# cadia-lvl/ss_asr

Measured on AMD Instinct MI355X. Metric: train-step utterances/sec on 80-dim mel, higher is better.
Workload: dtype f32; 1 GPU; BASELINE.json configs[1]: one ASRTrainer.exec iteration (GPU batch assembly from the HBM-resident corpus + engine.ASRTrainStep), ~10h synthetic Malromur-shape fbanks (8000 utts, <=800 frames, 80-dim), batch 32 per GPU, bucketed by length, LAS 256/256/128, tf_rate 0.9, Adadelta; global_batch=32, max_frames=800, parallelism=dp1, matrix_products=fp32 as 6 bf16 MFMAs on exact 3-way operand split, fp32 accumulate

## Files before the change

### ss_asr_amd/csrc/common.h

```cpp
#pragma once
#include <hip/hip_runtime.h>
#include <stdint.h>

typedef float f32x4 __attribute__((ext_vector_type(4)));

#define SSASR_OK 0
#define SSASR_EARG (-1)

#define SSASR_LAUNCH_CHECK()                         \
  do {                                               \
    hipError_t e__ = hipGetLastError();              \
    if (e__ != hipSuccess) return (int)e__;          \
  } while (0)

#define SSASR_HIP(call)                              \
  do {                                               \
    hipError_t e__ = (call);                         \
    if (e__ != hipSuccess) return (int)e__;          \
  } while (0)

struct RowMap {
  int64_t ld;
  int64_t inner;
  int64_t so;
// ... 130 lines not shown
  int no_fused_input;
  int bptt_halves_off;
  int bptt_reserve_kb;
  int no_persistent_decoder;
  int no_persistent_decoder_bwd;
  int delay_fwd, delay_bwd, delay_bwd_ksplit;
  int gemm_tile;
  int gemm_trace_lo, gemm_trace_hi;
  int gemm_wide;
  int gemm_bf16;
  int gemm_x6;
  int gemm_kcat;
  int no_windows;
  int bptt_one_launch;
  int wgrad_fused;
  int last_seg_pct;
  int tail_inline;
  int no_residency_check;
  int test_drop_tile;
  int test_drop_attn_slice;
  int test_drop_dec_slice;
  int attn_rph;
  int no_tsave;
};
const SsasrOptions& ssasr_options();
int64_t ssasr_resident_capacity(const void* kernel, int threads, size_t dyn_lds);
size_t ssasr_gemm_min_lds_bytes();
size_t ssasr_lds_reservation_against_gemm(const void* kernel);
bool ssasr_bptt_ksplit_ok(int64_t S, int64_t N, int64_t H, int dirs);
extern "C" int64_t ssasr_bilstm_bwd_gx_floats(int64_t S, int64_t N, int64_t H);
int ssasr_launch_colsum(const float* m, int64_t rows, int cols, int64_t ld, float* out, hipStream_t st,
                        float* out2 = nullptr);
```

### ss_asr_amd/csrc/decoder.hip

```cpp
#include "../../include/ssasr.h"
#include "attn_kernels.h"
#include "rnn_kernels.h"
#ifdef SSASR_TRACE_BUILD
constexpr int DTR_STEPS = 64, DTR_SLOTS = 8, DTR_WG = 256;
__device__ unsigned long long g_dtrace[DTR_WG * DTR_STEPS * DTR_SLOTS];
#define SSASR_DTRACE(step, slot) do { if (threadIdx.x == 0 && (step) < DTR_STEPS) { \
  unsigned long long t_; asm volatile("s_memrealtime %0\n\ts_waitcnt lgkmcnt(0)" : "=s"(t_) :: "memory"); \
  g_dtrace[(blockIdx.x * DTR_STEPS + (step)) * DTR_SLOTS + (slot)] = t_; } } while (0)
#endif
#include "decoder_persistent.h"
#include "decoder_long.h"
#include "decoder_bwd_persistent.h"
#include <cstdlib>

extern "C" int ssasr_abi_version(void) { return 16; }
#ifdef SSASR_TRACE_BUILD
extern "C" int ssasr_debug_dtrace(void* dst, size_t bytes) {
  SSASR_HIP(hipMemcpyFromSymbol(dst, HIP_SYMBOL(g_dtrace), bytes));
  return SSASR_OK;
}
#endif

extern "C" int64_t ssasr_decoder_bwd_chain_floats(int64_t U, int64_t B, int64_t T, int64_t A, int64_t E, int64_t D) {
  if (A != PD_A || E != PD_E || D != PD_D || B <= 0 || B > 32 || T <= 0 || U <= 0) return 0;
  if (chain_slices(T) == 0 || chain_slices(T) * B > CB_MAXATT) return 0;
  if (chain_xc_floats(U) * sizeof(float) >= (1ull << 31)) return 0;
  return (int64_t)(U * B * A + ((U * B + 63) & ~(int64_t)63) + chain_xa_floats(U) + chain_xc_floats(U) +
                   chain_xu_floats(U, T) + U * B * 4 * D);
}

namespace {
bool dec_grid_fits(const void* kernel, int threads, size_t dyn_lds, int64_t workgroups);
bool dec_long_taken(int64_t B, int64_t T, int64_t A, int64_t E, int64_t D, int64_t V) {
  const SsasrOptions& opt = ssasr_options();
  if (A != PD_A || E != PD_E || D != PD_D || V <= 0 || V > 64 || !pl_shape_ok(B, T)) return false;
  if (opt.no_persistent || opt.no_persistent_decoder) return false;
  const void* fn = reinterpret_cast<const void*>(decoder_fwd_long_kernel);
  if (hipFuncSetAttribute(fn, hipFuncAttributeMaxDynamicSharedMemorySize, (int)decoder_long_lds()) != hipSuccess) return false;
  return dec_grid_fits(fn, 512, decoder_long_lds(), (int64_t)pl_ns(T) * B + PL_NCMP);
}
}

extern "C" int64_t ssasr_decoder_fwd_part_floats(int64_t B, int64_t T, int64_t A, int64_t E, int64_t D, int64_t V) {
  return dec_long_taken(B, T, A, E, D, V) ? pl_part_floats(B, T) : 0;
}

extern "C" int ssasr_attn_precompute_fwd(const float* feat, const float* w_psi, const float* b_psi,
                                         int64_t rows, int64_t E, int64_t A, float* comp,
                                         void* stream) {
  if (!feat || !w_psi || !comp || rows <= 0 || E <= 0 || A <= 0) return SSASR_EARG;
  GemmDesc g{};
// ... 371 lines not shown
  int rc;
  const int64_t rows = U * B;
  const RowMap logit_rows{0, B, V, U * V};

  {
    GemmDesc m{};
    m.A = g.dlogits; m.ma = logit_rows;
    m.B = d.w_ct; m.mb = rm_dense(D);
    m.C = g.ws_dh2; m.mc = rm_dense(D);
    m.M = (int)rows; m.N = (int)D; m.K = (int)V; m.ta = 0; m.tb = 1;
    m.alpha = 1.f; m.beta = 0.f; m.splitk = 1; m.batch = 1;
    if ((rc = ssasr_launch_gemm(m, st))) return rc;
  }

  const bool cell2_first = g.ws_gx && g.ws_sync && ssasr_bilstm_bwd_gx_floats(U, B, D) > 0 &&
                           !opt.no_persistent && !opt.no_persistent_decoder;
  const bool cell2_direct = cell2_first && ssasr_bptt_ksplit_ok(U, B, D, 1);
  bool chain = cell2_first && g.ws_chain && ssasr_decoder_bwd_chain_floats(U, B, T, A, E, D) > 0 &&
               !opt.no_persistent_decoder_bwd;
  const int nsl = chain_slices(T);
  const void* chain_fn = nsl == 6 ? reinterpret_cast<const void*>(decoder_bwd_chain_kernel<6>)
                       : nsl == 4 ? reinterpret_cast<const void*>(decoder_bwd_chain_kernel<4>)
                                  : reinterpret_cast<const void*>(decoder_bwd_chain_kernel<2>);
  if (chain) {
    const size_t lds = chain_lds_bytes((int)T);
    SSASR_HIP(hipFuncSetAttribute(chain_fn, hipFuncAttributeMaxDynamicSharedMemorySize, (int)lds));
    chain = dec_grid_fits(chain_fn, 320, lds, nsl * B + 64);
  }
  if (!chain) {
    if ((rc = ssasr_launch_transpose(d.w_phi, d.w_phi_t, (int)A, (int)D, st))) return rc;
    if ((rc = ssasr_launch_transpose(d.w_ih1, g.ws_t_ih1, (int)(4 * D), (int)(D + E), st))) return rc;
    if ((rc = ssasr_launch_transpose(d.w_hh1, g.ws_t_hh1, (int)(4 * D), (int)D, st))) return rc;
  }
  if (!cell2_first && (rc = ssasr_launch_transpose(d.w_ih2, g.ws_t_ih2, (int)(4 * D), (int)D, st))) return rc;
  if (!cell2_direct && (rc = ssasr_launch_transpose(d.w_hh2, g.ws_t_hh2, (int)(4 * D), (int)D, st))) return rc;

  dim3 cgrid = cell_bwd_grid(D, 1, B), cblock(256);
  float* dc1 = g.ws_dc;
  float* dc2 = g.ws_dc + 2 * B * D;
  if (cell2_first) {
    if ((rc = ssasr_launch_bptt_persistent(cell2_direct ? nullptr : g.ws_t_hh2, d.gates2, d.c2, g.ws_dh2, B * D, D,
                                           nullptr, g.ws_gx, g.ws_sync, U, B, D, 1, st, 0, 0, nullptr,
                                           cell2_direct ? d.w_hh2 : nullptr, nullptr, armed && cell2_direct)))
      return rc;
    GemmDesc m{};
    m.A = d.gates2; m.ma = rm_dense(4 * D);
    m.B = d.w_ih2; m.mb = rm_dense(D);
    m.C = g.ws_dh2; m.mc = rm_dense(D);
    m.M = (int)rows; m.N = (int)D; m.K = (int)(4 * D); m.ta = 0; m.tb = 1;
    m.alpha = 1.f; m.beta = 0.f; m.splitk = 1; m.batch = 1;
    if (((rows + 63) / 64) * ((D + 63) / 64) < 192) {
      SSASR_HIP(hipMemsetAsync(g.ws_dh2, 0, sizeof(float) * rows * D, st));
      m.splitk = 4;
    }
    if ((rc = ssasr_launch_gemm(m, st))) return rc;
  }
  if (chain) {
    float* wsV = g.ws_chain;
    float* wsS = wsV + U * B * A;
    float* xa = wsS + ((U * B + 63) & ~(int64_t)63);
    float* xc = xa + chain_xa_floats(U);
    float* xu = xc + chain_xc_floats(U);
    float* dg1 = xu + chain_xu_floats(U, T);
    {
      GemmDesc m{};
      m.A = d.att; m.ma = rm_dense(T); m.sa = U * T;
      m.B = d.comp; m.mb = rm_dense(A); m.sb = T * A;
      m.C = wsV; m.mc = rm_dense(B * A); m.sc = A;
      m.M = (int)U; m.N = (int)A; m.K = (int)T; m.ta = 0; m.tb = 1;
      m.alpha = 1.f; m.beta = 0.f; m.splitk = 1; m.batch = (int)B;
      if ((rc = ssasr_launch_gemm(m, st))) return rc;
    }
    if (!armed)
      SSASR_HIP(hipMemsetD32Async((hipDeviceptr_t)xa, (int)PERSIST_SENTINEL,
                                  chain_xa_floats(U) + chain_xc_floats(U) + chain_xu_floats(U, T), st));
    DecBwdChain c{};
    c.gates1 = d.gates1; c.dg1 = dg1; c.c1 = d.c1; c.add1 = g.ws_dh2; c.att = d.att; c.q = d.q; c.feat = d.feat;
    c.comp = d.comp; c.enc_len = d.enc_len; c.V = wsV; c.w_hh1 = d.w_hh1; c.w_ih1 = d.w_ih1;
    c.w_phi = d.w_phi; c.dctx = g.ws_dctx; c.de = g.ws_de; c.dqpre = g.ws_dqpre; c.ssum = wsS;
    c.xa = xa; c.xc = xc; c.xu = xu; c.status = g.ws_sync + 5;
    c.B = (int)B; c.T = (int)T; c.U = (int)U;
    const size_t lds = chain_lds_bytes((int)T);
    const dim3 cgrid_chain((unsigned)(nsl * B + 64));
    if (nsl == 6) hipLaunchKernelGGL(decoder_bwd_chain_kernel<6>, cgrid_chain, dim3(320), lds, st, c);
    else if (nsl == 4) hipLaunchKernelGGL(decoder_bwd_chain_kernel<4>, cgrid_chain, dim3(320), lds, st, c);
    else hipLaunchKernelGGL(decoder_bwd_chain_kernel<2>, cgrid_chain, dim3(320), lds, st, c);
    hipLaunchKernelGGL(chain_de_fixup_kernel, dim3(256), dim3(256), 0, st, g.ws_de, d.att, wsS, (int)B, (int)U, (int)T,
                       reinterpret_cast<float4*>(d.gates1), reinterpret_cast<const float4*>(dg1), U * B * D,
                       g.ws_dqpre, (int)(B * A));
    SSASR_LAUNCH_CHECK();
  }
  for (int64_t t = U - 1; t >= 0 && !chain; --t) {
    const int64_t i = U - 1 - t;
    const bool last = (t == U - 1);
    CellBwdPair p2{};
    if (!cell2_first) {
      CellBwd& c = p2.d[0];
      int ns = 0;
      if (!last) {
        seg_set(c.sl, ns++, d.gates2 + (t + 1) * B * 4 * D, 4 * D, g.ws_t_hh2, 4 * D, (int)(4 * D));
        c.dc_in = dc2 + (i & 1) * B * D;
      }
      c.sl.nseg = ns;
      c.add1 = g.ws_dh2 + t * B * D; c.ld1 = D;
      c.gates = d.gates2 + t * B * 4 * D; c.dgates = d.gates2 + t * B * 4 * D;
      c.c_prev = t ? d.c2 + (t - 1) * B * D : nullptr;
// ... 124 lines not shown
```

### ss_asr_amd/csrc/decoder_bwd_persistent.h

```cpp
#pragma once
#include "decoder_persistent.h"

namespace {

constexpr int CB_XU_SLOTS = 34;
constexpr int CB_MAXATT = 192;
__host__ __device__ inline int cb_xu_step(int nsl) { return 2 * nsl * CB_XU_SLOTS * 16 * 4; }
__host__ __device__ inline int chain_slices(int64_t T) { return T <= 128 ? 2 : T <= 256 ? 4 : T <= 384 ? 6 : 0; }

struct DecBwdChain {
  const float* gates1;
  float* dg1;
  const float* c1;
  const float* add1;
  const float* att;
  const float* q;
  const float* feat;
  const float* comp;
  const int32_t* enc_len;
  const float* V;
  const float* w_hh1;
  const float* w_ih1;
  const float* w_phi;
  float* dctx;
  float* de;
  float* dqpre;
  float* ssum;
  float* xa;
  float* xc;
  float* xu;
  int* status;
  int B, T, U;
};

__host__ __device__ inline size_t chain_xa_floats(int64_t U) { return (size_t)U * 2 * 16 * 16 * 256; }
__host__ __device__ inline size_t chain_xc_floats(int64_t U) { return (size_t)U * 2 * 16 * 32 * 256; }
__host__ __device__ inline size_t chain_xu_floats(int64_t U, int64_t T) { return (size_t)U * cb_xu_step(chain_slices(T)); }
inline size_t chain_lds_bytes(int T) {
  const int nsl = chain_slices(T);
  const size_t att = ((size_t)((T + nsl - 1) / nsl) * PD_E + PD_E + 8 * PD_A + 16) * sizeof(float);
  const size_t cell = (4 * 64 * 4 + 2 * 7 * 64 * 4 + 4 * 64 * 4 + 8 * 4 * 16 * 4) * sizeof(float);
  return att > cell ? att : cell;
}

__global__ void chain_de_fixup_kernel(float* de, const float* att, const float* ssum, int B, int U, int T,
                                      float4* gates1, const float4* dg1, int64_t ng4, float* dqpre0, int nq) {
  const int64_t tid = blockIdx.x * (int64_t)blockDim.x + threadIdx.x, nth = (int64_t)gridDim.x * blockDim.x;
  for (int64_t i = tid; i < ng4; i += nth) gates1[i] = dg1[i];
  for (int64_t i = tid; i < nq; i += nth) dqpre0[i] = 0.f;
  const int64_t n = (int64_t)B * U * T;
  for (int64_t i = tid; i < n; i += nth) {
    const int64_t b = i / ((int64_t)U * T);
    const int64_t t = (i / T) % U;
    de[i] = t > 0 ? de[i] - att[i] * ssum[t * B + b] : 0.f;
  }
}

#ifndef SSASR_WPACE_UP
#define SSASR_WPACE_UP 12
#endif
#ifndef SSASR_WPACE_CLEAN
#define SSASR_WPACE_CLEAN 2
#endif
#ifndef SSASR_WPACE_DOWN
#define SSASR_WPACE_DOWN 2
#endif
#ifndef SSASR_WPACE_INIT
#define SSASR_WPACE_INIT 100
#endif
#ifndef SSASR_WPACE_INIT_ATT
#define SSASR_WPACE_INIT_ATT 120
#endif
struct WavePacer {
  int delay, clean;
  __device__ __forceinline__ void sleep() const {
    for (int k = 0; k < delay; ++k) __builtin_amdgcn_s_sleep(1);
  }
  __device__ __forceinline__ void update(bool missed) {
#ifdef SSASR_CHAIN_NO_PACE
    delay = 0; return;
#endif
    if (missed) { delay = min(delay + SSASR_WPACE_UP, 400); clean = 0; }
    else if (++clean >= SSASR_WPACE_CLEAN) { delay = max(delay - SSASR_WPACE_DOWN, 0); clean = 0; }
  }
};

template <int NV, typename F>
__device__ __forceinline__ bool cb_fetch(u32x4 (&raw)[NV], F ld, int* status) {
#pragma unroll
  for (int j = 0; j < NV; ++j) raw[j] = ld(j);
  bool missed = false;
  for (unsigned tries = 0;; ++tries) {
    bool anybad = false;
#pragma unroll
    for (int j = 0; j < NV; ++j) {
      const bool bad = raw[j].x == PERSIST_SENTINEL || raw[j].y == PERSIST_SENTINEL ||
                       raw[j].z == PERSIST_SENTINEL || raw[j].w == PERSIST_SENTINEL;
      if (__any(bad)) {
        anybad = true;
        raw[j] = ld(j);
      }
    }
    if (!anybad) break;
    missed = true;
    if (persist_give_up(tries, status, persist_code(PK_DEC_CHAIN, 0xfff))) break;
    __builtin_amdgcn_s_sleep(2);
  }
  return missed;
}

template <int NV, typename F>
__device__ __forceinline__ bool cb_verify(u32x4 (&raw)[NV], F ld, int* status) {
  bool missed = false;
  for (unsigned tries = 0;; ++tries) {
    bool anybad = false;
#pragma unroll
    for (int j = 0; j < NV; ++j) {
      const bool bad = raw[j].x == PERSIST_SENTINEL || raw[j].y == PERSIST_SENTINEL ||
                       raw[j].z == PERSIST_SENTINEL || raw[j].w == PERSIST_SENTINEL;
      if (__any(bad)) {
        anybad = true;
        raw[j] = ld(j);
      }
    }
    if (!anybad) break;
    missed = true;
    if (persist_give_up(tries, status, persist_code(PK_DEC_CHAIN, 0xfff))) break;
    __builtin_amdgcn_s_sleep(2);
  }
  return missed;
}

template <int NSL>
__global__ __launch_bounds__(320) void decoder_bwd_chain_kernel(DecBwdChain p) {
  extern __shared__ __attribute__((aligned(16))) float smem[];
  const int tid = threadIdx.x, wave = tid >> 6, lane = tid & 63;
  const int B = p.B, T = p.T, U = p.U;
  constexpr int D = PD_D, E = PD_E, A = PD_A;
  const __amdgpu_buffer_rsrc_t rxa = pd_rsrc(p.xa, chain_xa_floats(U) * sizeof(float));
  const __amdgpu_buffer_rsrc_t rxc = pd_rsrc(p.xc, chain_xc_floats(U) * sizeof(float));
  const __amdgpu_buffer_rsrc_t rxu = pd_rsrc(p.xu, chain_xu_floats(U, T) * sizeof(float));
  constexpr unsigned TILE_B = 64 * 16;
  constexpr unsigned XA_STEP = 2u * 16 * 16 * TILE_B, XC_STEP = 2u * 16 * 32 * TILE_B;
  constexpr int CB_XU_STEP = 2 * NSL * CB_XU_SLOTS * 16 * 4;
  const int natt = NSL * B;

  if ((int)blockIdx.x < natt) {
    const int b = (int)blockIdx.x / NSL, th = (int)blockIdx.x - b * NSL;
    if (wave == 4) return;
    const int Th = (T + NSL - 1) / NSL;
    const int tau0 = th * Th;
    int len = p.enc_len ? p.enc_len[b] : T;
    len = len < T ? len : T;
    const int nrow = max(0, min(len, tau0 + Th) - tau0);
    float* sF = smem;
    float* sD = sF + (size_t)Th * E;
    float* sRed = sD + E;
    float* sS = sRed + 8 * A;
    const float* fb = p.feat + ((int64_t)b * T + tau0) * E;
    lds_fill_quads<256>(sF, fb, nrow * (E / 4), tid);
    __syncthreads();
    const int c = b >> 4, bl = b & 15;
    const int cq = tid & 127, sh = tid >> 7;
    const int hw = tid >> 5, l32 = tid & 31;
    const float* cb = p.comp + ((int64_t)b * T + tau0) * A + 4 * l32;
    constexpr int RPG = 8;
    float4 cvr[RPG];
#pragma unroll
// ... 93 lines not shown
          for (int g = 0; g < 8; ++g) v.x += sS[g];
        }
        pd_st_sc1(rxu, (unsigned)(t * CB_XU_STEP + ((((c * NSL + th) * CB_XU_SLOTS + lane) * 16 + bl) * 4)) * 4u, v);
      }
      SSASR_DTRACE(U - 1 - t, 3);
      __syncthreads();
    }
    return;
  }

  const int cidx = (int)blockIdx.x - natt;
  const int tile = cidx >> 2, chunk = (cidx >> 1) & 1, half = cidx & 1;
  const int r = lane & 15, q = lane >> 4;
  const int n0 = 16 * chunk;
  const int n = n0 + r;
  const bool col_ok = n < B;
  const int u0 = 16 * tile + 4 * q;
  f32x4* red = reinterpret_cast<f32x4*>(smem);
  float4* coef = reinterpret_cast<float4*>(smem + 4 * 64 * 4);
  float4* sG = coef + 2 * 7 * 64;
  float4* sQ = sG + 4 * 64;

  if (wave == 4) {
    EncPersistBwd e{};
    e.dy = p.add1; e.ys_s = B * D; e.ys_n = D; e.S = U; e.N = B; e.H = D;
    BpttSaved sv;
    if (col_ok) {
      sv.fetch(e, p.gates1, p.c1, 0, 0, n, u0);
      sv.publish(&coef[(0 & 1) * 7 * 64 + lane], true);
      if (U > 1) sv.fetch(e, p.gates1, p.c1, 0, 1, n, u0);
    }
    for (int i = 0; i < U; ++i) {
      __syncthreads();
      if (col_ok && i + 1 < U) {
        sv.publish(&coef[((i + 1) & 1) * 7 * 64 + lane], true);
        if (i + 2 < U) sv.fetch(e, p.gates1, p.c1, 0, i + 2, n, u0);
      }
      __syncthreads();
      __syncthreads();
    }
    return;
  }

  float4 wa[2][4], wc[4][4], wp[2];
#pragma unroll
  for (int t = 0; t < 2; ++t) {
    const int unit = 16 * (half * 8 + 2 * wave + t) + r;
#pragma unroll
    for (int g = 0; g < 4; ++g) {
      const float* w = p.w_hh1 + (int64_t)(g * D + 16 * tile + 4 * q) * D + unit;
      wa[t][g] = make_float4(w[0], w[D], w[2 * D], w[3 * D]);
    }
  }
#pragma unroll
  for (int t = 0; t < 4; ++t) {
    const int col = 16 * (half * 16 + 4 * wave + t) + r;
#pragma unroll
    for (int g = 0; g < 4; ++g) {
      const float* w = p.w_ih1 + (int64_t)(g * D + 16 * tile + 4 * q) * (D + E) + D + col;
// ... 253 lines not shown
```

### ss_asr_amd/csrc/options.hip

```cpp
#include <cstdlib>
#include <cstring>
#include <map>
#include <mutex>
#include <tuple>
#include "../../include/ssasr.h"
#include "common.h"

namespace {

SsasrOptions g_opt;
std::once_flag g_opt_once;

int env_int(const char* name, int dflt) {
  const char* v = getenv(name);
  return v ? atoi(v) : dflt;
}
int env_flag(const char* name) { return getenv(name) != nullptr; }

void init_options() {
  g_opt.no_persistent = env_flag("SSASR_NO_PERSISTENT");
  g_opt.no_fused_input = env_flag("SSASR_NO_FUSED_INPUT");
  g_opt.bptt_halves_off = env_flag("SSASR_BPTT_HALVES_OFF");
  g_opt.bptt_reserve_kb = env_flag("SSASR_BPTT_SHARED_CU") ? 0 : env_int("SSASR_BPTT_RESERVE_KB", 118);
  g_opt.no_persistent_decoder = env_flag("SSASR_NO_PERSISTENT_DECODER");
  g_opt.no_persistent_decoder_bwd = env_flag("SSASR_NO_PERSISTENT_DECODER_BWD");
  g_opt.delay_fwd = env_int("SSASR_PERSIST_DELAY_FWD", -1);
  g_opt.delay_bwd = env_int("SSASR_PERSIST_DELAY_BWD", -1);
  g_opt.delay_bwd_ksplit = g_opt.delay_bwd;
  g_opt.gemm_tile = env_int("SSASR_GEMM_TILE", 0);
  g_opt.gemm_x6 = env_int("SSASR_GEMM_X6", 1);
  g_opt.gemm_wide = env_int("SSASR_GEMM_WIDE", 1);
  g_opt.gemm_bf16 = env_int("SSASR_GEMM_BF16", 0);
  g_opt.gemm_trace_lo = g_opt.gemm_trace_hi = 0;
  g_opt.gemm_kcat = env_int("SSASR_GEMM_KCAT", 1);
  g_opt.wgrad_fused = env_int("SSASR_WGRAD_FUSED", 1);
  g_opt.bptt_one_launch = env_int("SSASR_BPTT_ONE_LAUNCH", 1);
  g_opt.no_windows = env_flag("SSASR_NO_WINDOWS");
  g_opt.last_seg_pct = env_int("SSASR_LAST_SEG_PCT", 60);
  g_opt.tail_inline = env_int("SSASR_TAIL_INLINE", 1);
  g_opt.no_residency_check = env_flag("SSASR_NO_RESIDENCY_CHECK");
  g_opt.test_drop_tile = env_int("SSASR_TEST_DROP_TILE", -1);
  g_opt.test_drop_attn_slice = env_int("SSASR_TEST_DROP_ATTN_SLICE", -1);
  g_opt.test_drop_dec_slice = env_int("SSASR_TEST_DROP_DEC_SLICE", -1);
  g_opt.attn_rph = env_int("SSASR_ATTN_RPH", 0);
  if (g_opt.attn_rph != 2 && g_opt.attn_rph != 3 && g_opt.attn_rph != 4 && g_opt.attn_rph != 6) g_opt.attn_rph = 0;
  g_opt.no_tsave = env_flag("SSASR_NO_TSAVE");
}

struct Named { const char* name; int SsasrOptions::*field; };
const Named kNames[] = {
    {"SSASR_NO_PERSISTENT", &SsasrOptions::no_persistent},
    {"SSASR_NO_FUSED_INPUT", &SsasrOptions::no_fused_input},
    {"SSASR_BPTT_HALVES_OFF", &SsasrOptions::bptt_halves_off},
    {"SSASR_BPTT_RESERVE_KB", &SsasrOptions::bptt_reserve_kb},
    {"SSASR_NO_PERSISTENT_DECODER", &SsasrOptions::no_persistent_decoder},
    {"SSASR_NO_PERSISTENT_DECODER_BWD", &SsasrOptions::no_persistent_decoder_bwd},
    {"SSASR_PERSIST_DELAY_FWD", &SsasrOptions::delay_fwd},
    {"SSASR_PERSIST_DELAY_BWD", &SsasrOptions::delay_bwd},
    {"SSASR_GEMM_TILE", &SsasrOptions::gemm_tile},
    {"SSASR_GEMM_TRACE_LO", &SsasrOptions::gemm_trace_lo},
    {"SSASR_GEMM_TRACE_HI", &SsasrOptions::gemm_trace_hi},
    {"SSASR_GEMM_X6", &SsasrOptions::gemm_x6},
    {"SSASR_GEMM_WIDE", &SsasrOptions::gemm_wide},
    {"SSASR_GEMM_BF16", &SsasrOptions::gemm_bf16},
    {"SSASR_GEMM_KCAT", &SsasrOptions::gemm_kcat},
    {"SSASR_WGRAD_FUSED", &SsasrOptions::wgrad_fused},
    {"SSASR_BPTT_ONE_LAUNCH", &SsasrOptions::bptt_one_launch},
    {"SSASR_NO_WINDOWS", &SsasrOptions::no_windows},
    {"SSASR_LAST_SEG_PCT", &SsasrOptions::last_seg_pct},
    {"SSASR_TAIL_INLINE", &SsasrOptions::tail_inline},
    {"SSASR_NO_RESIDENCY_CHECK", &SsasrOptions::no_residency_check},
    {"SSASR_TEST_DROP_TILE", &SsasrOptions::test_drop_tile},
    {"SSASR_TEST_DROP_ATTN_SLICE", &SsasrOptions::test_drop_attn_slice},
    {"SSASR_TEST_DROP_DEC_SLICE", &SsasrOptions::test_drop_dec_slice},
    {"SSASR_ATTN_RPH", &SsasrOptions::attn_rph},
    {"SSASR_NO_TSAVE", &SsasrOptions::no_tsave},
};

}

const SsasrOptions& ssasr_options() {
  std::call_once(g_opt_once, init_options);
  return g_opt;
}

extern "C" int ssasr_set_option(const char* name, int value) {
  if (!name) return SSASR_EARG;
  std::call_once(g_opt_once, init_options);
  for (const Named& n : kNames)
    if (strcmp(n.name, name) == 0) {
      g_opt.*(n.field) = value;
      if (n.field == &SsasrOptions::delay_bwd) g_opt.delay_bwd_ksplit = value;
      return SSASR_OK;
    }
  return SSASR_EARG;
}

extern "C" int ssasr_get_option(const char* name, int* value) {
  if (!name || !value) return SSASR_EARG;
  std::call_once(g_opt_once, init_options);
  for (const Named& n : kNames)
    if (strcmp(n.name, name) == 0) { *value = g_opt.*(n.field); return SSASR_OK; }
  return SSASR_EARG;
}

size_t ssasr_lds_reservation_against_gemm(const void* kernel) {
// ... 25 lines not shown
```

### ss_asr_amd/csrc/rnn_kernels.h

```cpp
#pragma once
#include "common.h"

#ifndef SSASR_PERSIST_PRIO
#define SSASR_PERSIST_PRIO 3
#endif
#ifndef SSASR_PTRACE
#define SSASR_PTRACE(step, slot)
#define SSASR_PTRACE_H(step, slot)
#define SSASR_PRETRY(tries)
#endif
#ifndef SSASR_STAMP
#define SSASR_STAMP(i)
#define SSASR_STAMP_DRAIN()
#else
#define SSASR_STAMP_DRAIN() asm volatile("s_waitcnt vmcnt(0)" ::: "memory")
#endif

namespace {

constexpr int MAXSEG = 3;

struct SegList {
  const float* X[MAXSEG];
  const float* W[MAXSEG];
// ... 275 lines not shown
  PersistRole r;
  r.nchunk = gridDim.z / hv;
  r.tile = (gridDim.x & 7) ? blockIdx.x : (blockIdx.x & 7) * (gridDim.x >> 3) + (blockIdx.x >> 3);
  r.d = blockIdx.y;
  r.chunk = blockIdx.z / hv;
  r.half = blockIdx.z % hv;
  return r;
}

__device__ __forceinline__ float4 ld4(const float* p) { return *reinterpret_cast<const float4*>(p); }

__device__ __forceinline__ int xcd_grouped_tile(int bx, int ntile) {
#ifdef SSASR_NO_TILE_GROUPING
  return bx;
#else
  return (ntile & 7) ? bx : (bx & 7) * (ntile >> 3) + (bx >> 3);
#endif
}

constexpr unsigned PERSIST_MAX_SPINS = 1u << 20;

constexpr unsigned PERSIST_SENTINEL = 0x7FC0DEADu;

enum { PK_ENC_FWD = 1, PK_ENC_BPTT = 2, PK_DEC_FWD = 4, PK_DEC_CHAIN = 5 };
__device__ __forceinline__ int persist_code(int kernel, int step) {
  const unsigned wg = blockIdx.x + gridDim.x * (blockIdx.y + gridDim.y * blockIdx.z);
  return (int)(0x40000000u | ((unsigned)kernel << 24) | ((wg & 0xfffu) << 12) | ((unsigned)step & 0xfffu));
}
__device__ __forceinline__ bool persist_give_up(unsigned tries, int* status, int code) {
  if (tries > PERSIST_MAX_SPINS) {
    if ((threadIdx.x & 63) == 0) atomicCAS(status, 0, code);
    return true;
  }
  return (tries & 255u) == 8u && __hip_atomic_load(status, __ATOMIC_RELAXED, __HIP_MEMORY_SCOPE_AGENT) != 0;
}

struct PersistPacer {
  int delay;
  int clean;
  __device__ __forceinline__ void sleep() const {
    for (int k = 0; k < delay; ++k) __builtin_amdgcn_s_sleep(1);
  }
#ifndef SSASR_PACE_UP
#define SSASR_PACE_UP 2
#endif
#ifndef SSASR_PACE_CLEAN
#define SSASR_PACE_CLEAN 2
// ... 490 lines not shown
#pragma unroll
    for (int k = 0; k < 4; ++k) {
      const float tc = fast_tanh(c_[k]);
      kA[k] = go_[k] * (1.f - tc * tc);
      kO[k] = live ? tc * go_[k] * (1.f - go_[k]) : 0.f;
      kI[k] = live ? gg_[k] * gi_[k] * (1.f - gi_[k]) : 0.f;
      kG[k] = live ? gi_[k] * (1.f - gg_[k] * gg_[k]) : 0.f;
      kF[k] = live ? cp_[k] * gf_[k] * (1.f - gf_[k]) : 0.f;
      kC[k] = live ? gf_[k] : 0.f;
    }
    c[0 * 64] = make_float4(kA[0], kA[1], kA[2], kA[3]);
    c[1 * 64] = make_float4(kO[0], kO[1], kO[2], kO[3]);
    c[2 * 64] = make_float4(kI[0], kI[1], kI[2], kI[3]);
    c[3 * 64] = make_float4(kG[0], kG[1], kG[2], kG[3]);
    c[4 * 64] = make_float4(kF[0], kF[1], kF[2], kF[3]);
    c[5 * 64] = make_float4(kC[0], kC[1], kC[2], kC[3]);
    c[6 * 64] = ad;
  }
};

__device__ __forceinline__ bool epi_rows_ok(bool col_ok, int half, int hv, bool inplace, int i, int i0) {
  return col_ok && half == 0 && (hv == 1 || !inplace || i >= i0 + 2);
}
template <int TPW, int HV>
__global__ __launch_bounds__(320) void lstm_enc_bwd_rs_kernel(EncPersistBwd e) {
  constexpr int NW = 4;
  if (SSASR_PERSIST_PRIO) __builtin_amdgcn_s_setprio(SSASR_PERSIST_PRIO);
  constexpr int T = 4 * TPW;
  constexpr int SPW = T / NW;
  constexpr int OT = (T / HV) / NW;
  constexpr int LAG = HV >= 2 ? 3 : 1;
  static_assert(TPW % HV == 0 && (T / HV) % NW == 0 && T % NW == 0 && OT >= 1 && LAG + 2 <= BWD_RS_RING, "ring too short");
  __shared__ __attribute__((aligned(16))) float4 coef[3][7][64];
  constexpr int NG = HV >= 2 ? 3 : 1;
  __shared__ __attribute__((aligned(16))) float4 sG[NG][4][64];
  __shared__ int missed;
  const int tid = threadIdx.x, wave = tid >> 6, lane = tid & 63;
  if (tid == 0) missed = 0;
  __syncthreads();
  const int r = lane & 15, q = lane >> 4;
  const PersistRole role = persist_role(HV);
  const int tile = role.tile, d = role.d, chunk = role.chunk, half = role.half;
  const int nchunk = role.nchunk;
  const bool inplace = e.tsave == nullptr;
  const int S = e.S, N = e.N, H = e.H;
  const int i0 = e.i0, i1 = e.i1 > 0 ? e.i1 : S;
  const int n0 = chunk * 16;
  const int NT = e.nt > 0 ? e.nt : N;
  const int64_t rows = (int64_t)S * NT;
  const int u0 = 16 * tile + 4 * q;
  const int n = n0 + r;
  const bool col_ok = n < N;
  float* gbase = e.gates + (int64_t)d * rows * 4 * H;
  const float* cbase = e.cs + (int64_t)d * rows * H;

  constexpr unsigned TILE_B = 64 * 16;
  constexpr unsigned SLOT_B = (unsigned)T * T * TILE_B;
  float* xbase = e.gx + ((int64_t)d * nchunk + chunk) * (BWD_RS_RING * (int64_t)(SLOT_B / 4));
  const __amdgpu_buffer_rsrc_t xrs =
      __builtin_amdgcn_make_buffer_rsrc(xbase, 0, (int)(BWD_RS_RING * SLOT_B), 0x00020000);

  if (wave == NW) {
    const int len = (col_ok && e.lens) ? e.lens[n] : 0x7fffffff;
    BpttSaved sv;
    auto live = [&](int i) { return (d ? i : S - 1 - i) < len; };
    if (col_ok) {
      sv.fetch(e, gbase, cbase, d, i0, n, u0);
      sv.publish(&coef[i0 % 3][0][lane], live(i0));
      if (i0 + 1 < S) {
        sv.fetch(e, gbase, cbase, d, i0 + 1, n, u0);
        sv.publish(&coef[(i0 + 1) % 3][0][lane], live(i0 + 1));
      }
      if (i0 + 2 < S) sv.fetch(e, gbase, cbase, d, i0 + 2, n, u0);
    }
    PersistPacer pacer{e.delay, 0};
    const u32x4 fill = {PERSIST_SENTINEL, PERSIST_SENTINEL, PERSIST_SENTINEL, PERSIST_SENTINEL};
    __syncthreads();
    int sig_k = -1, sig_stage = 0;
    for (int i = i0; i < i1; ++i) {
      if (i > 0) {
        if (i > i0) pacer.sleep();
        asm volatile("s_waitcnt vmcnt(0)" ::: "memory");
        if (sig_stage == 2) {
          asm volatile("buffer_wbl2 sc1" ::: "memory");
          sig_stage = 1;
        } else if (sig_stage == 1) {
          if (lane == 0) __hip_atomic_fetch_add(e.progress + sig_k, 1u, __ATOMIC_RELAXED, __HIP_MEMORY_SCOPE_SYSTEM);
          sig_stage = 0;
        }
        __syncthreads();
      }
      if (col_ok && i + 2 < S) {
        sv.publish(&coef[(i + 2) % 3][0][lane], live(i + 2));
        if (i + 3 < S) sv.fetch(e, gbase, cbase, d, i + 3, n, u0);
      }
      __syncthreads();
      if (epi_rows_ok(col_ok, half, HV, inplace, i, i0)) {
        const int sr = d ? i : S - 1 - i;
        float* g0 = gbase + ((int64_t)sr * NT + n) * 4 * H + u0;
#pragma unroll
        for (int g = 0; g < 4; ++g) st4(g0 + (int64_t)g * H, sG[i % NG][g][lane]);
      }
      if (e.nbound > 0 && half == 0) {
#pragma unroll
        for (int k = 0; k < 7; ++k)
          if (k < e.nbound && i + 1 == e.bound[k]) { sig_k = k; sig_stage = 2; }
      }
      if (i > i0) {
        pacer.update(missed != 0);
        missed = 0;
      }
      if (half == 0 && i >= LAG) {
        const unsigned base = (unsigned)((i - LAG) % BWD_RS_RING) * SLOT_B + (unsigned)tile * T * TILE_B;
#pragma unroll
        for (int j = 0; j < T; ++j) {
          __builtin_amdgcn_raw_buffer_store_b128(fill, xrs, (int)(j * TILE_B + lane * 16), (int)base, 16);
        }
      }
      if (HV >= 2 && inplace && half == 0 && col_ok && i == i0 + 2) {
#pragma unroll
        for (int k = 0; k < 2; ++k) {
          const int sr = d ? i0 + k : S - 1 - (i0 + k);
          float* g0 = gbase + ((int64_t)sr * NT + n) * 4 * H + u0;
#pragma unroll
          for (int g = 0; g < 4; ++g) st4(g0 + (int64_t)g * H, sG[(i0 + k) % NG][g][lane]);
// ... 43 lines not shown
    SSASR_PTRACE(i, 0);
    if (i > 0) {
      __syncthreads();
      SSASR_PTRACE(i, 2);
      const unsigned base = (unsigned)((i - 1) % BWD_RS_RING) * SLOT_B + (unsigned)tile * T * TILE_B;
      u32x4 raw[SPW];
      const unsigned lo = (unsigned)(q * TILE_B + (wave * 16 + r) * 16);
      constexpr unsigned LSTEP = 4 * TILE_B;
#pragma unroll
      for (int t = 0; t < SPW; ++t)
        raw[t] = __builtin_amdgcn_raw_buffer_load_b128(xrs, (int)(lo + t * LSTEP), (int)base, 16);
      for (unsigned tries = 0;; ++tries) {
        bool anybad = false;
#pragma unroll
        for (int t = 0; t < SPW; ++t) {
          const bool bad = raw[t].x == PERSIST_SENTINEL || raw[t].y == PERSIST_SENTINEL ||
                           raw[t].z == PERSIST_SENTINEL || raw[t].w == PERSIST_SENTINEL;
          if (__any(bad)) {
            anybad = true;
            raw[t] = __builtin_amdgcn_raw_buffer_load_b128(xrs, (int)(lo + t * LSTEP), (int)base, 16);
          }
        }
        if (!anybad) { SSASR_PRETRY(tries); if (tries && lane == 0) missed = 1; break; }
        if (persist_give_up(tries, e.status, persist_code(PK_ENC_BPTT, i))) break;
        __builtin_amdgcn_s_sleep(2);
      }
      SSASR_PTRACE(i, 3);
#pragma unroll
      for (int t = 0; t < SPW; ++t) part += __builtin_bit_cast(f32x4, raw[t]);
    }
    SSASR_PTRACE(i, 1);
    {
      float v4[4] = {part[0], part[1], part[2], part[3]};
#pragma unroll
      for (int k2 = 0; k2 < 4; ++k2) {
        float mine;
        const float other = swap16_other(v4[k2], mine);
        const float s2 = mine + other;
        const auto r32 = __builtin_amdgcn_permlane32_swap(__float_as_uint(s2), __float_as_uint(s2), false, false);
        v4[k2] = __uint_as_float(r32[0]) + __uint_as_float(r32[1]);
      }
      const float dh_in = q == 0 ? v4[0] : q == 1 ? v4[1] : q == 2 ? v4[2] : v4[3];
      SSASR_PTRACE(i, 4);
      SSASR_PTRACE(i, 5);
      const int el = 16 * wave + r;
      float di = 0.f, df = 0.f, dg = 0.f, dov = 0.f;
      if (col_ok) {
// ... 45 lines not shown
          }
          piece[kb] = __builtin_bit_cast(bf16x8, make_uint4(u[0], u[1], u[2], u[3]));
        }
#pragma unroll
        for (int pa = 0; pa + level < 3; ++pa) {
#pragma unroll
          for (int t = 0; t < OT; ++t) {
            acc[t] = __builtin_amdgcn_mfma_f32_16x16x32_bf16(wA[t][0][pa], piece[0], acc[t], 0, 0, 0);
            acc2[t] = __builtin_amdgcn_mfma_f32_16x16x32_bf16(wA[t][1][pa], piece[1], acc2[t], 0, 0, 0);
          }
        }
      }
      SSASR_PTRACE(i, 10);
      const unsigned base = (unsigned)(i % BWD_RS_RING) * SLOT_B + (unsigned)tile * TILE_B;
#pragma unroll
      for (int t = 0; t < OT; ++t) {
        __builtin_amdgcn_raw_buffer_store_b128(__builtin_bit_cast(u32x4, acc[t] + acc2[t]), xrs,
                                               (int)((otile0 + t) * T * TILE_B + lane * 16), (int)base, 16);
      }
      SSASR_PTRACE(i, 7);
    }
  }
  if (col_ok && half == 0 && i1 < S && dcs1) *dcs1 = dc1;
}

struct PlainMm {
  SegList sl;
  float* out;
  int ldo;
  int N, R;
  int act;
};

__global__ __launch_bounds__(256) void seg_matmul_plain_kernel(PlainMm pa) {
  const PlainMm a = pa;
  __shared__ __attribute__((aligned(16))) f32x4 red[4 * BWD_NB * 64];
  const int tile = blockIdx.x;
  const int n0 = blockIdx.z * (16 * BWD_NB);
  const int lane = threadIdx.x & 63;
  const int r = lane & 15, q = lane >> 4;
  const int urow = 16 * tile + r;
  seg_matmul_tile<BWD_NB, BWD_UN>(a.sl, urow, urow < a.R, n0, a.N, red);
  const int bt = threadIdx.x >> 6;
  if (bt >= BWD_NB) return;
  const int n = n0 + 16 * bt + r;
  if (n >= a.N) return;
// ... 104 lines not shown
```

### ss_asr_amd/ops.py

```python
import ctypes as C
import os
import weakref

import torch

from . import _lib
from ._lib import check


_persist_status = []
TIMEOUT_MESSAGE = 'ss_asr_amd: a persistent recurrence / decode loop timed out'
_KERNELS = {1: 'encoder forward recurrence', 2: 'encoder BPTT',
            4: 'decode loop forward', 5: 'decoder backward chain', 6: 'split-T attention step'}


def describe_status(words):
    parts = []
    for v in words:
        v = int(v) & 0xffffffff
        if v == 0:
            continue
        if v & 0x40000000:
            step = v & 0xfff
            parts.append('%s, workgroup %d, %s' % (_KERNELS.get((v >> 24) & 0x3f, 'kernel %d' % ((v >> 24) & 0x3f)),
                                                    (v >> 12) & 0xfff, 'step %d' % step if step != 0xfff else 'step unknown'))
        else:
            parts.append('status %d' % v)
    return TIMEOUT_MESSAGE + (' (' + '; '.join(parts) + ')' if parts else '')


def check_persistent_status():
    global _persist_status
    pending, _persist_status = _persist_status, []
    if pending:
        words = torch.stack([t[i] for t, i in pending]).cpu().tolist()
        if any(words):
# ... 1012 lines not shown
```

Measured before the change: 5578 utterances/sec.

## Run decoder second-cell BPTT as wavefront roles inside the backward chain kernel

Instead of running the decoder's second LSTM cell BPTT as a separate persistent kernel before the backward chain, the chain kernel gains extra workgroups. Some act as cell-2 BPTT roles that publish per-step gate gradients, and others are bridge roles that multiply those gradients by w_ih2 to form the add1 input. The cell-1 chain consumes these step by step through sentinel-polled buffers, so the two recurrences overlap in a wavefront instead of running back to back. This costs extra workgroups and workspace, adds cross-workgroup spin-waiting, and requires the whole larger grid to be co-resident. It is enabled by default when the slice count is 2 and the grid fits.

```diff
diff --git a/ss_asr_amd/csrc/common.h b/ss_asr_amd/csrc/common.h
--- a/ss_asr_amd/csrc/common.h
+++ b/ss_asr_amd/csrc/common.h
@@ -176,7 +176,10 @@
   int test_drop_dec_slice;
   int attn_rph;
   int no_tsave;
+  int dec_bwd_wavefront;
+  int dec_bwd_last_form;
 };
+void ssasr_note_dec_bwd_form(int form);
 const SsasrOptions& ssasr_options();
 int64_t ssasr_resident_capacity(const void* kernel, int threads, size_t dyn_lds);
 size_t ssasr_gemm_min_lds_bytes();
diff --git a/ss_asr_amd/csrc/decoder.hip b/ss_asr_amd/csrc/decoder.hip
--- a/ss_asr_amd/csrc/decoder.hip
+++ b/ss_asr_amd/csrc/decoder.hip
@@ -11,6 +11,7 @@
 #include "decoder_persistent.h"
 #include "decoder_long.h"
 #include "decoder_bwd_persistent.h"
+#include <algorithm>
 #include <cstdlib>
 
 extern "C" int ssasr_abi_version(void) { return 16; }
@@ -26,7 +27,7 @@
   if (chain_slices(T) == 0 || chain_slices(T) * B > CB_MAXATT) return 0;
   if (chain_xc_floats(U) * sizeof(float) >= (1ull << 31)) return 0;
   return (int64_t)(U * B * A + ((U * B + 63) & ~(int64_t)63) + chain_xa_floats(U) + chain_xc_floats(U) +
-                   chain_xu_floats(U, T) + U * B * 4 * D);
+                   chain_xu_floats(U, T) + chain_xg_floats(U, B) + chain_xd_floats(U, B) + U * B * 4 * D);
 }
 
 namespace {
@@ -444,11 +445,15 @@
   const void* chain_fn = nsl == 6 ? reinterpret_cast<const void*>(decoder_bwd_chain_kernel<6>)
                        : nsl == 4 ? reinterpret_cast<const void*>(decoder_bwd_chain_kernel<4>)
                                   : reinterpret_cast<const void*>(decoder_bwd_chain_kernel<2>);
+  bool wavefront = false;
   if (chain) {
     const size_t lds = chain_lds_bytes((int)T);
     SSASR_HIP(hipFuncSetAttribute(chain_fn, hipFuncAttributeMaxDynamicSharedMemorySize, (int)lds));
-    chain = dec_grid_fits(chain_fn, 320, lds, nsl * B + 64);
-  }
+    wavefront = opt.dec_bwd_wavefront && nsl == 2 && cell2_direct && U >= 3 && !opt.bptt_halves_off &&
+                dec_grid_fits(chain_fn, 320, lds, nsl * B + 64 + CB_NCELL2 + CB_NBRIDGE);
+    chain = wavefront || dec_grid_fits(chain_fn, 320, lds, nsl * B + 64);
+  }
+  ssasr_note_dec_bwd_form(wavefront ? 2 : chain ? 1 : 0);
   if (!chain) {
     if ((rc = ssasr_launch_transpose(d.w_phi, d.w_phi_t, (int)A, (int)D, st))) return rc;
     if ((rc = ssasr_launch_transpose(d.w_ih1, g.ws_t_ih1, (int)(4 * D), (int)(D + E), st))) return rc;
@@ -460,7 +465,7 @@
   dim3 cgrid = cell_bwd_grid(D, 1, B), cblock(256);
   float* dc1 = g.ws_dc;
   float* dc2 = g.ws_dc + 2 * B * D;
-  if (cell2_first) {
+  if (cell2_first && !wavefront) {
     if ((rc = ssasr_launch_bptt_persistent(cell2_direct ? nullptr : g.ws_t_hh2, d.gates2, d.c2, g.ws_dh2, B * D, D,
                                            nullptr, g.ws_gx, g.ws_sync, U, B, D, 1, st, 0, 0, nullptr,
                                            cell2_direct ? d.w_hh2 : nullptr, nullptr, armed && cell2_direct)))
@@ -483,7 +488,9 @@
     float* xa = wsS + ((U * B + 63) & ~(int64_t)63);
     float* xc = xa + chain_xa_floats(U);
     float* xu = xc + chain_xc_floats(U);
-    float* dg1 = xu + chain_xu_floats(U, T);
+    float* xg = xu + chain_xu_floats(U, T);
+    float* xd = xg + chain_xg_floats(U, B);
+    float* dg1 = xd + chain_xd_floats(U, B);
     {
       GemmDesc m{};
       m.A = d.att; m.ma = rm_dense(T); m.sa = U * T;
@@ -493,17 +500,28 @@
       m.alpha = 1.f; m.beta = 0.f; m.splitk = 1; m.batch = (int)B;
       if ((rc = ssasr_launch_gemm(m, st))) return rc;
     }
-    if (!armed)
+    if (!armed) {
       SSASR_HIP(hipMemsetD32Async((hipDeviceptr_t)xa, (int)PERSIST_SENTINEL,
-                                  chain_xa_floats(U) + chain_xc_floats(U) + chain_xu_floats(U, T), st));
+                                  chain_xa_floats(U) + chain_xc_floats(U) + chain_xu_floats(U, T) +
+                                      (wavefront ? chain_xg_floats(U, B) + chain_xd_floats(U, B) : 0), st));
+      if (wavefront)
+        SSASR_HIP(hipMemsetD32Async((hipDeviceptr_t)g.ws_gx, (int)PERSIST_SENTINEL,
+                                    (size_t)ssasr_bilstm_bwd_ring_floats(U, B, D, 1), st));
+    }
     DecBwdChain c{};
     c.gates1 = d.gates1; c.dg1 = dg1; c.c1 = d.c1; c.add1 = g.ws_dh2; c.att = d.att; c.q = d.q; c.feat = d.feat;
     c.comp = d.comp; c.enc_len = d.enc_len; c.V = wsV; c.w_hh1 = d.w_hh1; c.w_ih1 = d.w_ih1;
     c.w_phi = d.w_phi; c.dctx = g.ws_dctx; c.de = g.ws_de; c.dqpre = g.ws_dqpre; c.ssum = wsS;
     c.xa = xa; c.xc = xc; c.xu = xu; c.status = g.ws_sync + 5;
     c.B = (int)B; c.T = (int)T; c.U = (int)U;
+    if (wavefront) {
+      c.add1 = nullptr;
+      c.gates2 = d.gates2; c.c2 = d.c2; c.dh2 = g.ws_dh2; c.w_hh2 = d.w_hh2; c.w_ih2 = d.w_ih2;
+      c.gx2 = g.ws_gx; c.xg = xg; c.xd = xd;
+      c.delay2 = opt.delay_bwd_ksplit < 0 ? 40 : std::min(opt.delay_bwd_ksplit, 96);
+    }
     const size_t lds = chain_lds_bytes((int)T);
-    const dim3 cgrid_chain((unsigned)(nsl * B + 64));
+    const dim3 cgrid_chain((unsigned)(nsl * B + 64 + (wavefront ? CB_NCELL2 + CB_NBRIDGE : 0)));
     if (nsl == 6) hipLaunchKernelGGL(decoder_bwd_chain_kernel<6>, cgrid_chain, dim3(320), lds, st, c);
     else if (nsl == 4) hipLaunchKernelGGL(decoder_bwd_chain_kernel<4>, cgrid_chain, dim3(320), lds, st, c);
     else hipLaunchKernelGGL(decoder_bwd_chain_kernel<2>, cgrid_chain, dim3(320), lds, st, c);
diff --git a/ss_asr_amd/csrc/decoder_bwd_persistent.h b/ss_asr_amd/csrc/decoder_bwd_persistent.h
--- a/ss_asr_amd/csrc/decoder_bwd_persistent.h
+++ b/ss_asr_amd/csrc/decoder_bwd_persistent.h
@@ -31,7 +31,17 @@
   float* xu;
   int* status;
   int B, T, U;
+  float* gates2;
+  const float* c2;
+  const float* dh2;
+  const float* w_hh2;
+  const float* w_ih2;
+  float* gx2;
+  float* xg;
+  float* xd;
+  int delay2;
 };
+constexpr int CB_NCELL2 = 64, CB_NBRIDGE = 16;
 
 __host__ __device__ inline size_t chain_xa_floats(int64_t U) { return (size_t)U * 2 * 16 * 16 * 256; }
 __host__ __device__ inline size_t chain_xc_floats(int64_t U) { return (size_t)U * 2 * 16 * 32 * 256; }
@@ -40,8 +50,12 @@
   const int nsl = chain_slices(T);
   const size_t att = ((size_t)((T + nsl - 1) / nsl) * PD_E + PD_E + 8 * PD_A + 16) * sizeof(float);
   const size_t cell = (4 * 64 * 4 + 2 * 7 * 64 * 4 + 4 * 64 * 4 + 8 * 4 * 16 * 4) * sizeof(float);
-  return att > cell ? att : cell;
-}
+  const size_t cell2 = (size_t)(3 * 7 * 64 + bptt_rs_ng(2) * 4 * 64) * sizeof(float4) + 16;
+  const size_t roles = cell > cell2 ? cell : cell2;
+  return att > roles ? att : roles;
+}
+__host__ __device__ inline size_t chain_xg_floats(int64_t U, int64_t B) { return (size_t)U * B * 4 * PD_D; }
+__host__ __device__ inline size_t chain_xd_floats(int64_t U, int64_t B) { return (size_t)U * B * PD_D; }
 
 __global__ void chain_de_fixup_kernel(float* de, const float* att, const float* ssum, int B, int U, int T,
                                       float4* gates1, const float4* dg1, int64_t ng4, float* dqpre0, int nq) {
@@ -86,7 +100,8 @@
 };
 
 template <int NV, typename F>
-__device__ __forceinline__ bool cb_fetch(u32x4 (&raw)[NV], F ld, int* status) {
+__device__ __forceinline__ bool cb_fetch(u32x4 (&raw)[NV], F ld, int* status,
+                                         int code = persist_code(PK_DEC_CHAIN, 0xfff)) {
 #pragma unroll
   for (int j = 0; j < NV; ++j) raw[j] = ld(j);
   bool missed = false;
@@ -103,14 +118,15 @@
     }
     if (!anybad) break;
     missed = true;
-    if (persist_give_up(tries, status, persist_code(PK_DEC_CHAIN, 0xfff))) break;
+    if (persist_give_up(tries, status, code)) break;
     __builtin_amdgcn_s_sleep(2);
   }
   return missed;
 }
 
 template <int NV, typename F>
-__device__ __forceinline__ bool cb_verify(u32x4 (&raw)[NV], F ld, int* status) {
+__device__ __forceinline__ bool cb_verify(u32x4 (&raw)[NV], F ld, int* status,
+                                          int code = persist_code(PK_DEC_CHAIN, 0xfff)) {
   bool missed = false;
   for (unsigned tries = 0;; ++tries) {
     bool anybad = false;
@@ -125,10 +141,81 @@
     }
     if (!anybad) break;
     missed = true;
-    if (persist_give_up(tries, status, persist_code(PK_DEC_CHAIN, 0xfff))) break;
+    if (persist_give_up(tries, status, code)) break;
     __builtin_amdgcn_s_sleep(2);
   }
   return missed;
+}
+
+__device__ __noinline__ void chain_bridge_role(const DecBwdChain& p, int j) {
+  extern __shared__ __attribute__((aligned(16))) float smem[];
+  const int tid = threadIdx.x, wave = tid >> 6, lane = tid & 63, r = lane & 15, q = lane >> 4;
+  if (wave == 4) return;
+  constexpr int D = PD_D;
+  const int B = p.B, U = p.U;
+  const __amdgpu_buffer_rsrc_t rg = pd_rsrc(p.xg, chain_xg_floats(U, B) * sizeof(float));
+  const __amdgpu_buffer_rsrc_t rd = pd_rsrc(p.xd, chain_xd_floats(U, B) * sizeof(float));
+  float4 w[16];
+#pragma unroll
+  for (int kk = 0; kk < 16; ++kk) {
+    const float* wp = p.w_ih2 + (int64_t)(256 * wave + 16 * kk + 4 * q) * D + 16 * j + r;
+    w[kk] = make_float4(wp[0], wp[D], wp[2 * D], wp[3 * D]);
+  }
+  f32x4* red = reinterpret_cast<f32x4*>(smem);
+  for (int t = U - 1; t >= 0; --t) {
+    const int code = persist_code(PK_DEC_CHAIN_BRIDGE, U - 1 - t);
+    for (int c = 0; c < 2; ++c) {
+      f32x4 acc = f32x4{0.f, 0.f, 0.f, 0.f}, acc2 = f32x4{0.f, 0.f, 0.f, 0.f};
+      if (16 * c < B) {
+        const int n = 16 * c + r;
+        const bool ok = n < B;
+        const unsigned base = (unsigned)((((int64_t)t * B + (ok ? n : 0)) * 4 * D + 256 * wave + 4 * q) * 4);
+        u32x4 raw[16];
+        cb_fetch<16>(raw, [=](int kk) { return ok ? pd_ld_raw(rg, base + (unsigned)kk * 64u) : u32x4{0u, 0u, 0u, 0u}; },
+                     p.status, code);
+#pragma unroll
+        for (int kk = 0; kk < 16; kk += 2) {
+          const f32x4 b0 = __builtin_bit_cast(f32x4, raw[kk]), b1 = __builtin_bit_cast(f32x4, raw[kk + 1]);
+          acc = __builtin_amdgcn_mfma_f32_16x16x4f32(w[kk].x, b0[0], acc, 0, 0, 0);
+          acc2 = __builtin_amdgcn_mfma_f32_16x16x4f32(w[kk + 1].x, b1[0], acc2, 0, 0, 0);
+          acc = __builtin_amdgcn_mfma_f32_16x16x4f32(w[kk].y, b0[1], acc, 0, 0, 0);
+          acc2 = __builtin_amdgcn_mfma_f32_16x16x4f32(w[kk + 1].y, b1[1], acc2, 0, 0, 0);
+          acc = __builtin_amdgcn_mfma_f32_16x16x4f32(w[kk].z, b0[2], acc, 0, 0, 0);
+          acc2 = __builtin_amdgcn_mfma_f32_16x16x4f32(w[kk + 1].z, b1[2], acc2, 0, 0, 0);
+          acc = __builtin_amdgcn_mfma_f32_16x16x4f32(w[kk].w, b0[3], acc, 0, 0, 0);
+          acc2 = __builtin_amdgcn_mfma_f32_16x16x4f32(w[kk + 1].w, b1[3], acc2, 0, 0, 0);
+        }
+      }
+      red[(c * 4 + wave) * 64 + lane] = acc + acc2;
+    }
+    __syncthreads();
+    if (wave < 2) {
+      const int n = 16 * wave + r;
+      if (n < B) {
+        const f32x4 v = (red[(wave * 4 + 0) * 64 + lane] + red[(wave * 4 + 1) * 64 + lane]) +
+                        (red[(wave * 4 + 2) * 64 + lane] + red[(wave * 4 + 3) * 64 + lane]);
+        __builtin_amdgcn_raw_buffer_store_b128(__builtin_bit_cast(u32x4, v), rd,
+                                               (int)((unsigned)((((int64_t)t * B + n) * D + 16 * j + 4 * q) * 4)), 0, 16);
+      }
+    }
+    __syncthreads();
+  }
+}
+
+__device__ __noinline__ void chain_cell2_role(const DecBwdChain& p, int k) {
+  extern __shared__ __attribute__((aligned(16))) float smem[];
+  constexpr int D = PD_D;
+  const int B = p.B, U = p.U;
+  PersistRole role;
+  role.tile = k >> 2; role.d = 0; role.chunk = (k >> 1) & 1; role.half = k & 1; role.nchunk = (B + 15) >> 4;
+  if (role.chunk >= role.nchunk) return;
+  EncPersistBwd e{};
+  e.gates = p.gates2; e.cs = p.c2; e.dy = p.dh2; e.gx = p.gx2; e.status = p.status; e.delay = p.delay2;
+  e.ys_s = B * D; e.ys_n = D; e.S = U; e.N = B; e.H = D; e.whh[0] = p.w_hh2;
+  float4(*coef2)[7][64] = reinterpret_cast<float4(*)[7][64]>(smem);
+  float4(*sG2)[4][64] = reinterpret_cast<float4(*)[4][64]>(smem + 3 * 7 * 64 * 4);
+  int* missed2 = reinterpret_cast<int*>(smem + (3 * 7 * 64 + bptt_rs_ng(2) * 4 * 64) * 4);
+  bptt_rs_role<4, 2>(e, role, coef2, sG2, missed2, p.xg, PK_DEC_CHAIN_CELL2);
 }
 
 template <int NSL>
@@ -144,6 +231,15 @@
   constexpr unsigned XA_STEP = 2u * 16 * 16 * TILE_B, XC_STEP = 2u * 16 * 32 * TILE_B;
   constexpr int CB_XU_STEP = 2 * NSL * CB_XU_SLOTS * 16 * 4;
   const int natt = NSL * B;
+
+  if constexpr (NSL == 2) {
+    if ((int)blockIdx.x >= natt + 64) {
+      const int k = (int)blockIdx.x - natt - 64;
+      if (k >= CB_NCELL2) { chain_bridge_role(p, k - CB_NCELL2); return; }
+      chain_cell2_role(p, k);
+      return;
+    }
+  }
 
   if ((int)blockIdx.x < natt) {
     const int b = (int)blockIdx.x / NSL, th = (int)blockIdx.x - b * NSL;
@@ -283,19 +379,36 @@
   float4* sQ = sG + 4 * 64;
 
   if (wave == 4) {
+    const bool wf = NSL == 2 && p.xd != nullptr;
+    const __amdgpu_buffer_rsrc_t rd = pd_rsrc(p.xd, wf ? chain_xd_floats(U, B) * sizeof(float) : 0);
     EncPersistBwd e{};
-    e.dy = p.add1; e.ys_s = B * D; e.ys_n = D; e.S = U; e.N = B; e.H = D;
+    e.dy = wf ? p.c1 : p.add1; e.ys_s = B * D; e.ys_n = D; e.S = U; e.N = B; e.H = D;
     BpttSaved sv;
+    u32x4 adr[1] = {u32x4{0u, 0u, 0u, 0u}};
+    auto ad_off = [=](int i) { return (unsigned)((((int64_t)(U - 1 - i) * B + n) * D + u0) * 4); };
+    auto fetch = [&](int i) {
+      sv.fetch(e, p.gates1, p.c1, 0, i, n, u0);
+      if (wf) adr[0] = pd_ld_raw(rd, ad_off(i));
+    };
+    auto publish = [&](int i) {
+      if (wf) {
+        const unsigned off = ad_off(i);
+        cb_verify<1>(adr, [=](int) { return pd_ld_raw(rd, off); }, p.status);
+        const f32x4 a = __builtin_bit_cast(f32x4, adr[0]);
+        sv.ad = make_float4(a[0], a[1], a[2], a[3]);
+      }
+      sv.publish(&coef[(i & 1) * 7 * 64 + lane], true);
+    };
     if (col_ok) {
-      sv.fetch(e, p.gates1, p.c1, 0, 0, n, u0);
-      sv.publish(&coef[(0 & 1) * 7 * 64 + lane], true);
-      if (U > 1) sv.fetch(e, p.gates1, p.c1, 0, 1, n, u0);
+      fetch(0);
+      publish(0);
+      if (U > 1) fetch(1);
     }
     for (int i = 0; i < U; ++i) {
       __syncthreads();
       if (col_ok && i + 1 < U) {
-        sv.publish(&coef[((i + 1) & 1) * 7 * 64 + lane], true);
-        if (i + 2 < U) sv.fetch(e, p.gates1, p.c1, 0, i + 2, n, u0);
+        publish(i + 1);
+        if (i + 2 < U) fetch(i + 2);
       }
       __syncthreads();
       __syncthreads();
diff --git a/ss_asr_amd/csrc/options.hip b/ss_asr_amd/csrc/options.hip
--- a/ss_asr_amd/csrc/options.hip
+++ b/ss_asr_amd/csrc/options.hip
@@ -45,6 +45,8 @@
   g_opt.attn_rph = env_int("SSASR_ATTN_RPH", 0);
   if (g_opt.attn_rph != 2 && g_opt.attn_rph != 3 && g_opt.attn_rph != 4 && g_opt.attn_rph != 6) g_opt.attn_rph = 0;
   g_opt.no_tsave = env_flag("SSASR_NO_TSAVE");
+  g_opt.dec_bwd_wavefront = 1;
+  g_opt.dec_bwd_last_form = 0;
 }
 
 struct Named { const char* name; int SsasrOptions::*field; };
@@ -75,6 +77,8 @@
     {"SSASR_TEST_DROP_DEC_SLICE", &SsasrOptions::test_drop_dec_slice},
     {"SSASR_ATTN_RPH", &SsasrOptions::attn_rph},
     {"SSASR_NO_TSAVE", &SsasrOptions::no_tsave},
+    {"SSASR_DEC_BWD_WAVEFRONT", &SsasrOptions::dec_bwd_wavefront},
+    {"SSASR_DEC_BWD_LAST_FORM", &SsasrOptions::dec_bwd_last_form},
 };
 
 }
@@ -82,6 +86,11 @@
 const SsasrOptions& ssasr_options() {
   std::call_once(g_opt_once, init_options);
   return g_opt;
+}
+
+void ssasr_note_dec_bwd_form(int form) {
+  std::call_once(g_opt_once, init_options);
+  g_opt.dec_bwd_last_form = form;
 }
 
 extern "C" int ssasr_set_option(const char* name, int value) {
diff --git a/ss_asr_amd/csrc/rnn_kernels.h b/ss_asr_amd/csrc/rnn_kernels.h
--- a/ss_asr_amd/csrc/rnn_kernels.h
+++ b/ss_asr_amd/csrc/rnn_kernels.h
@@ -321,7 +321,7 @@
 
 constexpr unsigned PERSIST_SENTINEL = 0x7FC0DEADu;
 
-enum { PK_ENC_FWD = 1, PK_ENC_BPTT = 2, PK_DEC_FWD = 4, PK_DEC_CHAIN = 5 };
+enum { PK_ENC_FWD = 1, PK_ENC_BPTT = 2, PK_DEC_FWD = 4, PK_DEC_CHAIN = 5, PK_DEC_CHAIN_CELL2 = 7, PK_DEC_CHAIN_BRIDGE = 8 };
 __device__ __forceinline__ int persist_code(int kernel, int step) {
   const unsigned wg = blockIdx.x + gridDim.x * (blockIdx.y + gridDim.y * blockIdx.z);
   return (int)(0x40000000u | ((unsigned)kernel << 24) | ((wg & 0xfffu) << 12) | ((unsigned)step & 0xfffu));
@@ -858,24 +858,22 @@
 __device__ __forceinline__ bool epi_rows_ok(bool col_ok, int half, int hv, bool inplace, int i, int i0) {
   return col_ok && half == 0 && (hv == 1 || !inplace || i >= i0 + 2);
 }
+__host__ __device__ constexpr int bptt_rs_ng(int hv) { return hv >= 2 ? 3 : 1; }
 template <int TPW, int HV>
-__global__ __launch_bounds__(320) void lstm_enc_bwd_rs_kernel(EncPersistBwd e) {
+__device__ __forceinline__ void bptt_rs_role(const EncPersistBwd& e, const PersistRole role, float4 (*coef)[7][64],
+                                             float4 (*sG)[4][64], int* missedp, float* pub, int pk) {
   constexpr int NW = 4;
-  if (SSASR_PERSIST_PRIO) __builtin_amdgcn_s_setprio(SSASR_PERSIST_PRIO);
   constexpr int T = 4 * TPW;
   constexpr int SPW = T / NW;
   constexpr int OT = (T / HV) / NW;
   constexpr int LAG = HV >= 2 ? 3 : 1;
   static_assert(TPW % HV == 0 && (T / HV) % NW == 0 && T % NW == 0 && OT >= 1 && LAG + 2 <= BWD_RS_RING, "ring too short");
-  __shared__ __attribute__((aligned(16))) float4 coef[3][7][64];
-  constexpr int NG = HV >= 2 ? 3 : 1;
-  __shared__ __attribute__((aligned(16))) float4 sG[NG][4][64];
-  __shared__ int missed;
+  constexpr int NG = bptt_rs_ng(HV);
+  int& missed = *missedp;
   const int tid = threadIdx.x, wave = tid >> 6, lane = tid & 63;
   if (tid == 0) missed = 0;
   __syncthreads();
   const int r = lane & 15, q = lane >> 4;
-  const PersistRole role = persist_role(HV);
   const int tile = role.tile, d = role.d, chunk = role.chunk, half = role.half;
   const int nchunk = role.nchunk;
   const bool inplace = e.tsave == nullptr;
@@ -895,6 +893,9 @@
   float* xbase = e.gx + ((int64_t)d * nchunk + chunk) * (BWD_RS_RING * (int64_t)(SLOT_B / 4));
   const __amdgpu_buffer_rsrc_t xrs =
       __builtin_amdgcn_make_buffer_rsrc(xbase, 0, (int)(BWD_RS_RING * SLOT_B), 0x00020000);
+
+  const __amdgpu_buffer_rsrc_t prs =
+      __builtin_amdgcn_make_buffer_rsrc(pub, 0, pub ? (int)(rows * 4 * H * sizeof(float)) : 0, 0x00020000);
 
   if (wave == NW) {
     const int len = (col_ok && e.lens) ? e.lens[n] : 0x7fffffff;
@@ -937,6 +938,14 @@
 #pragma unroll
         for (int g = 0; g < 4; ++g) st4(g0 + (int64_t)g * H, sG[i % NG][g][lane]);
       }
+      if (pub && col_ok && half == 0) {
+        const int sr = d ? i : S - 1 - i;
+        const unsigned off = (unsigned)((((int64_t)sr * NT + n) * 4 * H + u0) * 4);
+#pragma unroll
+        for (int g = 0; g < 4; ++g)
+          __builtin_amdgcn_raw_buffer_store_b128(__builtin_bit_cast(u32x4, sG[i % NG][g][lane]), prs,
+                                                 (int)(off + (unsigned)(g * H) * 4u), 0, 16);
+      }
       if (e.nbound > 0 && half == 0) {
 #pragma unroll
         for (int k = 0; k < 7; ++k)
@@ -1026,7 +1035,7 @@
           }
         }
         if (!anybad) { SSASR_PRETRY(tries); if (tries && lane == 0) missed = 1; break; }
-        if (persist_give_up(tries, e.status, persist_code(PK_ENC_BPTT, i))) break;
+        if (persist_give_up(tries, e.status, persist_code(pk, i))) break;
         __builtin_amdgcn_s_sleep(2);
       }
       SSASR_PTRACE(i, 3);
@@ -1118,6 +1127,15 @@
     }
   }
   if (col_ok && half == 0 && i1 < S && dcs1) *dcs1 = dc1;
+}
+
+template <int TPW, int HV>
+__global__ __launch_bounds__(320) void lstm_enc_bwd_rs_kernel(EncPersistBwd e) {
+  if (SSASR_PERSIST_PRIO) __builtin_amdgcn_s_setprio(SSASR_PERSIST_PRIO);
+  __shared__ __attribute__((aligned(16))) float4 coef[3][7][64];
+  __shared__ __attribute__((aligned(16))) float4 sG[bptt_rs_ng(HV)][4][64];
+  __shared__ int missed;
+  bptt_rs_role<TPW, HV>(e, persist_role(HV), coef, sG, &missed, nullptr, PK_ENC_BPTT);
 }
 
 struct PlainMm {
diff --git a/ss_asr_amd/ops.py b/ss_asr_amd/ops.py
--- a/ss_asr_amd/ops.py
+++ b/ss_asr_amd/ops.py
@@ -11,7 +11,8 @@
 _persist_status = []
 TIMEOUT_MESSAGE = 'ss_asr_amd: a persistent recurrence / decode loop timed out'
 _KERNELS = {1: 'encoder forward recurrence', 2: 'encoder BPTT',
-            4: 'decode loop forward', 5: 'decoder backward chain', 6: 'split-T attention step'}
+            4: 'decode loop forward', 5: 'decoder backward chain', 6: 'split-T attention step',
+            7: 'decoder backward chain (second-cell BPTT role)', 8: 'decoder backward chain (add1 bridge role)'}
 
 
 def describe_status(words):
```

Result: slower. 4859 utterances/sec (-12.9%).
